# ria8651/octree-tracer

Measured on AMD Instinct MI355X. Metric: Mrays/sec at 1920x1080, depth-16 SVO; achieved HBM GB/s vs peak, higher is better.
Workload: dtype f32+u32

## Files before the change

octree-tracer_amd/csrc/svo_abi.cpp:

```cpp
#include <hip/hip_runtime.h>

#include <cmath>
#include <cstdio>
#include <cstring>
#include <new>
#include <string>
#include <vector>

#include "svo_ctx.h"

int svo_fail(svo_ctx *ctx, int code, const char *what) {
    if (ctx) ctx->err = what;
    return code;
}

int svo_fail_hip(svo_ctx *ctx, hipError_t e, const char *what) {
    if (ctx) ctx->err = std::string(what) + ": " + hipGetErrorString(e);
    return SVO_ERR_HIP;
}

namespace {

constexpr size_t kScanCapacity = 1024000;

// ... 4 lines not shown
    do {                                                     \
        hipError_t e_ = (expr);                              \
        if (e_ != hipSuccess) return fail_hip(ctx, e_, #expr); \
    } while (0)

int bind(svo_ctx *ctx) {
    HIP_TRY(ctx, hipSetDevice(ctx->device));
    return SVO_OK;
}

int order_after_last_write(svo_ctx *ctx) {
    svo_node_store *st = ctx->store;
    if (st->last_write && st->last_writer != ctx->stream) HIP_TRY(ctx, hipStreamWaitEvent(ctx->stream, st->last_write, 0));
    return SVO_OK;
}

int note_write(svo_ctx *ctx, bool on_stream) {
    svo_node_store *st = ctx->store;
    st->version++;
    if (on_stream) {
        if (!st->last_write) HIP_TRY(ctx, hipEventCreateWithFlags(&st->last_write, hipEventDisableTiming));
        HIP_TRY(ctx, hipEventRecord(st->last_write, ctx->stream));
        st->last_writer = ctx->stream;
    }
    return SVO_OK;
}

void release_store(svo_ctx *ctx) {
    svo_node_store *st = ctx->store;
    ctx->store = nullptr;
    ctx->nodes = nullptr;
    ctx->capacity = 0;
    ctx->top_version = 0;
    if (!st || --st->refs > 0) return;
    (void)hipSetDevice(st->device);
    if (st->nodes && st->owned) (void)hipFree(st->nodes);
    if (st->last_write) (void)hipEventDestroy(st->last_write);
    delete st;
}

void adopt_store(svo_ctx *ctx, svo_node_store *st) {
    ctx->store = st;
    ctx->nodes = st->nodes;
    ctx->capacity = st->capacity;
    ctx->top_version = 0;
}

int ensure_top_table(svo_ctx *ctx) {
    if (ctx->top_version == ctx->store->version) return SVO_OK;
    int rc = order_after_last_write(ctx);
    if (rc) return rc;
    HIP_TRY(ctx, svo::launch_build_top_table(ctx->nodes, (uint32_t)ctx->capacity, ctx->top_table, ctx->stream));
    ctx->top_version = ctx->store->version;
    return SVO_OK;
}

bool cull_worthwhile(const svo_ctx *ctx) {
    if (ctx->cull_mode == 0) return false;
    const float *ci = ctx->uniforms.camera_inverse;
    const double w = ci[15];
    if (!(fabs(w) > 1e-20)) return false;
    const double o[3] = {ci[12] / w, ci[13] / w, ci[14] / w};
    if (!(fabs(o[0]) > 1.001 || fabs(o[1]) > 1.001 || fabs(o[2]) > 1.001)) return false;
    if (ctx->cull_mode == 1) return true;
    constexpr int NX = 12, NY = 8;
    int miss = 0;
    for (int j = 0; j < NY; j++)
        for (int i = 0; i < NX; i++) {
            const double cx = (i + 0.5) / NX * 2.0 - 1.0, cy = -((j + 0.5) / NY * 2.0 - 1.0);
            double d4[4];
            for (int r = 0; r < 4; r++) d4[r] = ci[r] * cx + ci[4 + r] * cy + ci[8 + r] + ci[12 + r];
            if (!(fabs(d4[3]) > 1e-20)) return false;
            double t0 = -1e300, t1 = 1e300;
            for (int k = 0; k < 3; k++) {
                const double d = d4[k] / d4[3] - o[k];
                if (d == 0.0) {
                    if (fabs(o[k]) > 1.0) t1 = -1e300;
                    continue;
// ... 12 lines not shown
    bool count_rays = false;
    int sched_slot = 0;
    const uint8_t *skip = nullptr;
    svo_hit *shadow_out = nullptr;
};

int trace_launch(svo_ctx *ctx, const svo::WorkDesc &work, const float *rays, svo_hit *hits, const TraceOpts &opt) {
    int rc = bind(ctx);
    if (rc) return rc;
    const bool want_stack = ctx->variant != SVO_VARIANT_RESTART && ctx->tree_depth <= (uint32_t)svo::stack_max_depth(true);
    if (want_stack) {
        rc = ensure_top_table(ctx);
        if (rc) return rc;
    } else {
        rc = order_after_last_write(ctx);
        if (rc) return rc;
    }
    svo::WorkDesc wd = work;
    auto magic = [](uint32_t d) -> uint32_t { return d <= 1u ? 0u : (uint32_t)(0x100000000ull / d) + 1u; };
    wd.magic_bpr = magic(wd.bpr);
    wd.magic_bprect = magic(wd.bprect);
    wd.magic_tiles_x = magic(wd.tiles_x);
    svo::TraceArgs a{};
    a.nodes = ctx->nodes;
    a.n_words = (uint32_t)ctx->capacity;
    a.top_table = ctx->top_table;
    a.u = ctx->uniforms;
    a.work = wd;
    a.rays = rays;
    a.hits = hits;
    a.aux_t = opt.aux_t;
    a.status = ctx->status;
    a.refill_min = ctx->refill_min;
    a.cam_shortcut = ctx->cam_shortcut ? 1u : 0u;
    a.debug = ctx->debug_buf;
    a.skip = opt.skip;
    const bool counting = (work.mode != 2 || opt.count_rays) && !(ctx->uniforms.flags & SVO_F_PAUSE_ADAPTIVE);
    a.count_nodes = counting ? ctx->nodes : nullptr;
    const bool debug_hits = (ctx->uniforms.flags & SVO_F_PAUSE_ADAPTIVE) && (ctx->uniforms.flags & SVO_F_SHOW_HITS);
    const bool stack = want_stack && !debug_hits;
    a.shadow_hits = stack ? opt.shadow_out : nullptr;
    const uint32_t n_strips = (wd.n_items + 63u) / 64u;
    const bool schedule = ctx->schedule && n_strips <= svo::kMaxScheduledStrips;
    svo_ctx::Sched &sc = ctx->sched[opt.sched_slot & 1];
    const bool cull = stack && schedule && wd.mode != 2 && hits != nullptr && cull_worthwhile(ctx);
    const bool filtered = stack && schedule && (opt.skip != nullptr || cull);
    if (stack && schedule) {
        if (sc.cap < n_strips) {
            HIP_TRY(ctx, hipStreamSynchronize(ctx->stream));
            if (sc.cost) (void)hipFree(sc.cost);
            if (sc.cls_now) (void)hipFree(sc.cls_now);
            if (sc.order) (void)hipFree(sc.order);
            if (sc.balance) (void)hipFree(sc.balance);
            sc = svo_ctx::Sched{};
            size_t want = n_strips < 4096 ? 4096 : n_strips;
            HIP_TRY(ctx, hipMalloc((void **)&sc.cost, want + 32 + svo::kOrderHistWords * sizeof(uint32_t)));
            HIP_TRY(ctx, hipMalloc((void **)&sc.cls_now, want + 32 + svo::kOrderHistWords * sizeof(uint32_t)));
            HIP_TRY(ctx, hipMalloc((void **)&sc.order, (2 * want + 8 * (svo::kCostClasses + 8) + 8) * sizeof(uint32_t)));
            HIP_TRY(ctx, hipMalloc((void **)&sc.balance, svo::kBalanceWords * sizeof(uint32_t)));
            sc.cap = want;
        }
        if (sc.valid && memcmp(&sc.key, &wd, sizeof(wd)) != 0) sc.valid = false;
        if (!sc.valid) {
            uint32_t init[svo::kBalanceWords] = {};
            for (uint32_t k = 0; k <= 8; k++) init[k] = k * 8192u;
            HIP_TRY(ctx, hipMemcpyAsync(sc.balance, init, sizeof(init), hipMemcpyHostToDevice, ctx->stream));
            sc.balance_frames = 0;
        }
        a.balance = ctx->list_balance ? sc.balance : nullptr;
        a.order_cap = svo::order_list_cap(wd, n_strips);
        if (filtered) {
            if (opt.skip)
                HIP_TRY(ctx, svo::launch_schedule_skipping(opt.skip, wd.n_items, sc.valid ? sc.cost : nullptr, sc.cls_now, sc.order, n_strips,
                                                           a.order_cap, ctx->stream));
            else
                HIP_TRY(ctx, svo::launch_schedule_culling(a, sc.valid ? sc.cost : nullptr, sc.cls_now, sc.order, n_strips, a.order_cap,
                                                          ctx->stream));
            a.order = sc.order;
            sc.order_filtered = true;
        } else {
            a.order = (sc.valid && !sc.order_filtered) ? sc.order : nullptr;
        }
    }
    svo::LaunchInfo li{};
    li.variant = stack ? SVO_VARIANT_STACK : SVO_VARIANT_RESTART;
    li.grid_blocks = ctx->grid_blocks;
    li.num_cus = ctx->num_cus;
    li.strip_items = ctx->strip_items;
    li.deep_stack = ctx->tree_depth > (uint32_t)svo::stack_max_depth(false);
    li.occupancy = ctx->occupancy;
    if (stack && ctx->defer_items < wd.n_items) {
        HIP_TRY(ctx, hipStreamSynchronize(ctx->stream));
        if (ctx->defer_buf) (void)hipFree(ctx->defer_buf);
        ctx->defer_buf = nullptr;
        ctx->frame_parity = 0;
        ctx->defer_items = 0;
        size_t want = wd.n_items < (1u << 16) ? (1u << 16) : wd.n_items;
        HIP_TRY(ctx, hipMalloc((void **)&ctx->defer_buf, (svo::kCounterWords + 2 * (want + 1)) * sizeof(uint32_t)));
        HIP_TRY(ctx, hipMemsetAsync(ctx->defer_buf, 0, (svo::kCounterWords + 2 * (want + 1)) * sizeof(uint32_t), ctx->stream));
        ctx->defer_items = want;
    }
    li.counters = ctx->defer_buf;
    li.work_counter = ctx->defer_buf;
    if (ctx->defer_buf) {
        uint32_t *lists = ctx->defer_buf + svo::kCounterWords;
        const size_t stride = ctx->defer_items + 1;
        li.defer = lists + (ctx->frame_parity ? stride : 0);
        li.next_defer_count = lists + (ctx->frame_parity ? 0 : stride);
    }
    const size_t slot = ctx->ev_slots ? (ctx->ev_count % ctx->ev_slots) : 0;
    const bool timed = ctx->ev_slots && opt.sched_slot == 0;
    if (timed) HIP_TRY(ctx, hipEventRecord(ctx->ev[2 * slot], ctx->stream));
    HIP_TRY(ctx, svo::launch_trace(a, li, ctx->stream));
    if (timed) {
        HIP_TRY(ctx, hipEventRecord(ctx->ev[2 * slot + 1], ctx->stream));
        ctx->ev_count++;
    }
    if (stack) {
        const bool same_input = (wd.mode != 2 || opt.sched_slot == 1) && sc.built_nodes_version == ctx->store->version &&
                                memcmp(&sc.built_uniforms, &ctx->uniforms, sizeof(svo_uniforms)) == 0 && sc.age < 64;
        const bool moving = sc.have_prev && memcmp(&sc.prev_uniforms, &ctx->uniforms, sizeof(svo_uniforms)) != 0;
        const bool fed_back = a.balance != nullptr && a.order != nullptr && !filtered;
        const bool rebuild = schedule && (!sc.valid || (sc.order_filtered && !filtered) || (!same_input && sc.age + 1 >= ctx->sched_period) ||
                                          (same_input && sc.floored && !moving) || (same_input && fed_back && sc.balance_frames < 16u));
        const bool shares_only = rebuild && sc.valid && same_input && fed_back && sc.balance_frames < 16u && !(sc.order_filtered && !filtered) &&
                                 !(sc.floored && !moving);
        const bool floor_now = rebuild && !filtered && moving && ctx->motion_floor != 0u && wd.mode == 0 && wd.n_rects == 1u;
        HIP_TRY(ctx, svo::launch_post(a, li, rebuild ? sc.cost : nullptr, sc.order, n_strips, svo::order_list_cap(wd, n_strips),
                                      rebuild && !filtered, ctx->stream, floor_now ? sc.cls_now : nullptr, ctx->motion_floor,
                                      (fed_back && (!same_input || sc.balance_frames < 16u)) ? sc.balance_frames + 1u : 0u, shares_only));
        if (fed_back) sc.balance_frames++;
        if (rebuild && !filtered) sc.floored = floor_now;
        sc.prev_uniforms = ctx->uniforms;
        sc.have_prev = true;
        ctx->frame_parity ^= 1;
        if (rebuild) {
            if (!filtered) sc.order_filtered = false;
            sc.key = wd;
            sc.valid = true;
            sc.age = 0;
            sc.built_uniforms = ctx->uniforms;
            sc.built_nodes_version = ctx->store->version;
        } else if (schedule) {
            sc.age++;
        }
    }
// ... 223 lines not shown
    HIP_TRY(ctx, hipStreamSynchronize(ctx->stream));
    if (ctx->comm_stream) HIP_TRY(ctx, hipStreamSynchronize(ctx->comm_stream));
    HIP_TRY(ctx, hipFree(device_ptr));
    return SVO_OK;
}

int svo_buffer_read(svo_ctx *ctx, const void *device_ptr, void *host_out, size_t bytes) {
    if (!ctx || ((!device_ptr || !host_out) && bytes)) return SVO_ERR_ARG;
    int rc = bind(ctx);
    if (rc || bytes == 0) return rc;
    HIP_TRY(ctx, hipMemcpyAsync(host_out, device_ptr, bytes, hipMemcpyDeviceToHost, ctx->stream));
    HIP_TRY(ctx, hipStreamSynchronize(ctx->stream));
    return SVO_OK;
}

int svo_ctx_create(int hip_device, svo_ctx **out) {
    if (!out) return SVO_ERR_ARG;
    *out = nullptr;
    int n = 0;
    if (hipGetDeviceCount(&n) != hipSuccess || n <= 0) return SVO_ERR_NO_DEVICE;
    if (hip_device < 0 || hip_device >= n) return SVO_ERR_ARG;
    svo_ctx *ctx = new (std::nothrow) svo_ctx();
    if (!ctx) return SVO_ERR_HIP;
    ctx->device = hip_device;
    hipError_t e = hipSetDevice(hip_device);
    hipDeviceProp_t prop;
    if (e == hipSuccess) e = hipGetDeviceProperties(&prop, hip_device);
    if (e == hipSuccess) {
        ctx->num_cus = prop.multiProcessorCount;
        e = hipStreamCreateWithFlags(&ctx->own_stream, hipStreamNonBlocking);
    }
    if (e == hipSuccess) e = hipMalloc((void **)&ctx->top_table, (svo::kTopEntries + svo::kTopAuxEntries) * sizeof(uint32_t));
    if (e == hipSuccess) e = hipMalloc((void **)&ctx->status, sizeof(uint32_t));
    if (e == hipSuccess) e = hipMemset(ctx->status, 0, sizeof(uint32_t));
    if (e != hipSuccess) {
        svo_ctx_destroy(ctx);
        return SVO_ERR_HIP;
    }
    ctx->stream = ctx->own_stream;
    *out = ctx;
    return SVO_OK;
}

int svo_ctx_destroy(svo_ctx *ctx) {
    if (!ctx) return SVO_OK;
    (void)hipSetDevice(ctx->device);
    if (ctx->stream) (void)hipStreamSynchronize(ctx->stream);
    svo_comm_release(ctx);
    release_store(ctx);
    if (ctx->top_table) (void)hipFree(ctx->top_table);
    if (ctx->status) (void)hipFree(ctx->status);
    if (ctx->defer_buf) (void)hipFree(ctx->defer_buf);
    for (auto &sc : ctx->sched) {
        if (sc.cost) (void)hipFree(sc.cost);
        if (sc.cls_now) (void)hipFree(sc.cls_now);
        if (sc.order) (void)hipFree(sc.order);
    }
    for (void *p : {ctx->shade_hits, ctx->shade_aux, ctx->shade_rays, ctx->shade_shadow, ctx->shade_skip, ctx->scatter_buf})
        if (p) (void)hipFree(p);
    if (ctx->scan_sub) (void)hipFree(ctx->scan_sub);
    if (ctx->stage) (void)hipFree(ctx->stage);
    for (hipEvent_t e : ctx->ev) (void)hipEventDestroy(e);
    if (ctx->own_stream) (void)hipStreamDestroy(ctx->own_stream);
    delete ctx;
    return SVO_OK;
}

int svo_ctx_set_stream(svo_ctx *ctx, void *hip_stream, int use_own) {
    if (!ctx) return SVO_ERR_ARG;
    int rc = bind(ctx);
    if (rc) return rc;
    HIP_TRY(ctx, hipStreamSynchronize(ctx->stream));
    ctx->stream = use_own ? ctx->own_stream : (hipStream_t)hip_stream;
    return SVO_OK;
}

int svo_set_option(svo_ctx *ctx, int option, int64_t value) {
    if (!ctx) return SVO_ERR_ARG;
    switch (option) {
        case SVO_OPT_VARIANT:
            if (value != SVO_VARIANT_RESTART && value != SVO_VARIANT_STACK) return fail(ctx, SVO_ERR_ARG, "unknown variant");
            ctx->variant = (int)value;
            return SVO_OK;
        case SVO_OPT_TIMING: {
// ... 445 lines not shown
```

octree-tracer_amd/csrc/svo_ctx.h:

```cpp
#pragma once
#include <cstdlib>
#include <hip/hip_runtime.h>

#include <cstdint>
#include <string>
#include <vector>

#include "svo_device.h"
#include "svo_hip.h"

struct svo_node_store {
    int device = 0;
    uint32_t *nodes = nullptr;
    size_t capacity = 0;
    bool owned = false;
    int refs = 1;
    uint64_t version = 1;
    hipEvent_t last_write = nullptr;
    hipStream_t last_writer = nullptr;
};

struct svo_ctx {
    int device = 0;
    int num_cus = 256;
    hipStream_t own_stream = nullptr;
    hipStream_t stream = nullptr;
    svo_node_store *store = nullptr;
    uint32_t *nodes = nullptr;
    size_t capacity = 0;
    uint64_t top_version = 0;
    uint32_t *top_table = nullptr;
    int cull_mode = 2;
    bool cam_shortcut = true;
    void *comm = nullptr;
    int comm_world = 0, comm_rank = 0;
    hipStream_t comm_stream = nullptr;
    hipEvent_t comm_ready = nullptr, comm_done = nullptr;
    bool gathers_issued = false;
    uint32_t *status = nullptr;
    uint32_t *defer_buf = nullptr;
    size_t defer_items = 0;
    uint32_t *scan_sub = nullptr, *scan_unsub = nullptr;
    size_t scan_capacity = 0;
    void *stage = nullptr;
    size_t stage_bytes = 0;
    svo_uniforms uniforms{};
    bool have_uniforms = false;
    int variant = SVO_VARIANT_STACK;
    int grid_blocks = 0;
    int occupancy[16] = {};
    uint32_t refill_min = 32;
    bool scan_clears = false;
    int fused_shadows = 2;
    void *scatter_buf = nullptr;
    size_t scatter_bytes = 0;
    uint32_t prio_steps = 0;
    uint32_t block_w_log2 = 3;
    uint32_t tree_depth = 16;
    struct Sched {
        uint8_t *cost = nullptr;
        uint8_t *cls_now = nullptr;
        uint32_t *order = nullptr;
        uint32_t *balance = nullptr;
        uint32_t balance_frames = 0;
        size_t cap = 0;
        bool valid = false;
// ... 30 lines not shown
```

octree-tracer_amd/csrc/svo_device.h:

```cpp
#pragma once
#include <hip/hip_runtime.h>
#include <stdint.h>

#include "svo_hip.h"

namespace svo {

constexpr uint32_t kVoxelOffset = 134217728u;
constexpr uint32_t kMaxDescent = 31;
constexpr int kTopLevels = 3;
constexpr int kTopEntries = 1 << (3 * kTopLevels);
constexpr int kTopAuxEntries = 8 + 64;
constexpr int kPathBits = 23;
#ifndef SVO_COUNTER_STRIDE
#define SVO_COUNTER_STRIDE 16416
#endif
constexpr int kCounterStride = SVO_COUNTER_STRIDE;
constexpr int kCounterWords = 64 * kCounterStride;


struct WorkDesc {
    uint32_t mode;
    uint32_t x0, y0;
    uint32_t w, h;
    uint32_t bw_log2;
    uint32_t bpr;
    uint32_t bprect;
    uint32_t n_rects;
    uint32_t tiles_x;
    uint32_t first_tile, tile_stride;
    uint32_t n_items;
    uint32_t magic_bpr, magic_bprect, magic_tiles_x;
};

struct TraceArgs {
    const uint32_t *nodes;
    uint32_t n_words;
    const uint32_t *top_table;
    svo_uniforms u;
    WorkDesc work;
    const float *rays;
    svo_hit *hits;
    uint32_t *rgba;
    float *aux_t;
    uint32_t *status;
    uint32_t refill_min;
    uint32_t cam_shortcut;
    uint32_t *count_nodes;
    const uint32_t *order;
    uint32_t order_cap;
    uint32_t *debug;
    const uint8_t *skip;
    uint32_t *balance;
    svo_hit *shadow_hits;
};

struct LaunchInfo {
    int variant;
    int grid_blocks;
    int num_cus;
    int *occupancy;
    bool deep_stack;
    uint32_t strip_items;
    uint32_t *counters;
    uint32_t *work_counter;
    uint32_t *defer;
    uint32_t *next_defer_count;
};

hipError_t launch_build_top_table(const uint32_t *nodes, uint32_t n_words, uint32_t *top_table,
                                  hipStream_t stream);
hipError_t launch_trace(const TraceArgs &args, const LaunchInfo &li, hipStream_t stream);
int stack_max_depth(bool deep);
constexpr uint32_t kMaxScheduledStrips = 1u << 20;
#ifndef SVO_COST_SHIFT
#define SVO_COST_SHIFT 2
#endif
constexpr uint32_t kCostShift = SVO_COST_SHIFT, kCostClasses = 128u >> SVO_COST_SHIFT;
constexpr uint32_t kOrderHistWords = 64 * kCostClasses;
constexpr uint32_t kBalanceHead = 32, kBalanceSlots = 4096, kBalanceWords = kBalanceHead + kBalanceSlots;
// ... 26 lines not shown
```

octree-tracer_amd/csrc/svo_kernels.hip:

```cpp
#include <hip/hip_runtime.h>

#include "svo_device.h"
#include "svo_trace_fn.h"

#ifndef SVO_WALK_STOP
#define SVO_WALK_STOP 1
#endif
#ifndef SVO_TOP_IN_LDS
#define SVO_TOP_IN_LDS 1
#endif
#ifndef SVO_WALK_TRIPS
#define SVO_WALK_TRIPS 1
#endif
#ifndef SVO_WALK_ASM
#define SVO_WALK_ASM 1
#endif
#ifndef SVO_WALK_LUT
#define SVO_WALK_LUT 2
#endif
#ifndef SVO_WALK_LUT_CNT
#define SVO_WALK_LUT_CNT 1
#endif
#ifndef SVO_DBG_LIGHT
#define SVO_DBG_LIGHT 0
#endif
#ifndef SVO_CAM_SCALAR
#define SVO_CAM_SCALAR 0
#endif
#ifndef SVO_WAVES_PER_SIMD_CNT
#define SVO_WAVES_PER_SIMD_CNT 6
#endif
#ifndef SVO_WAVES_PER_SIMD
#define SVO_WAVES_PER_SIMD 7
#endif

namespace svo {


__device__ __forceinline__ uint32_t count_add(uint32_t *nodes, uint32_t p, uint32_t word, uint32_t n) {
    while ((word & 15u) < 15u) {
        const uint32_t add = min(n, 15u - (word & 15u));
        const uint32_t seen = atomicCAS(&nodes[p], word, word + add);
        if (seen == word) return (word & 15u) + add;
        word = seen;
    }
    return 15u;
}

template <bool RUNS_ONLY = false>
__device__ __forceinline__ uint32_t visit_groups(uint32_t n_words, uint32_t p, uint32_t word) {
    const bool need = p < n_words && (word & 15u) < 15u;
    const uint64_t needmask = __ballot(need);
    if (!needmask) return 0u;
    const uint32_t lane = __lane_id();
    if (RUNS_ONLY) {
        const uint32_t pm = need ? p : 0xFFFFFFFFu;
        const uint32_t under = (uint32_t)__builtin_amdgcn_update_dpp(-1, (int)pm, 0x138, 0xF, 0xF, false);
        const bool head = need && under != pm;
        const uint64_t stop = ((((uint64_t)__ballot(head) | ~needmask) >> 1) | (1ull << 63)) >> lane;
        return head ? (uint32_t)__builtin_ctzll(stop) + 1u : 0u;
// ... 137 lines not shown
        entry = (((uint32_t)top_levels + 1u) << 27) | (tn & 0x07FFFFFFu);
    }
    table[cell] = entry;
    uint32_t at = (uint32_t)kTopEntries;
    for (int k = 1; k < top_levels; k++) {
        if (cell < (1u << (3 * k))) {
            const uint32_t kx = (cell >> (2 * k)) & ((1u << k) - 1u), ky = (cell >> k) & ((1u << k) - 1u), kz = cell & ((1u << k) - 1u);
            uint32_t g = 0;
            for (int lvl = 1; lvl <= k && g != 0xFFFFFFFFu; lvl++) {
                const int sh = k - lvl;
                const uint32_t child = (((kx >> sh) & 1u) << 2) | (((ky >> sh) & 1u) << 1) | ((kz >> sh) & 1u);
                const uint32_t tn = load_word(rs, g + child) >> 4;
                g = tn >= kVoxelOffset ? 0xFFFFFFFFu : tn;
            }
            table[at + cell] = g;
        }
        at += 1u << (3 * k);
    }
}


__device__ __forceinline__ const TraceArgs &fresh_args() {
    auto p = (const __attribute__((address_space(4))) char *)__builtin_amdgcn_kernarg_segment_ptr();
    asm volatile("" : "+s"(p));
    return *(const TraceArgs *)p;
}

template <int BLOCK, int NS, int K, bool CNT>
struct StackLds {
    static constexpr int top = SVO_TOP_IN_LDS != 0 ? (1 << (3 * K)) : 0;
    static constexpr int lut = top;
    static constexpr int pools = lut + 64;
    static constexpr int counting = pools + (BLOCK / 64) * (kPoolWords * 64);
    static constexpr int stacks = counting + (CNT ? (BLOCK / 64) * kCountQueue + kSatTags + (1 << (3 * K)) / 8 : 0);
    static constexpr int total = stacks + NS * BLOCK;
};
#if defined(__HIP_DEVICE_COMPILE__) && !defined(__gfx950__)
#error "svo_kernels.hip is written for gfx950: the walk relies on its handling of LDS accesses beyond the allocation and on v_rcp_f32 + one Newton step being the IEEE reciprocal (tools/rcptest_gpu.hip)"
#endif

template <int BLOCK, int NS, int K, bool GE, bool DBG, bool CNT, bool SHD>
__global__ __launch_bounds__(BLOCK, NS > 12 ? 4 : (CNT ? SVO_WAVES_PER_SIMD_CNT : ((SHD || (DBG && SVO_DBG_LIGHT == 0)) ? 6 : SVO_WAVES_PER_SIMD))) void trace_stack_kernel(TraceArgs a, uint32_t strip_items,
                                                               uint32_t *work_counter, uint32_t *defer) {
    constexpr bool DBGH = DBG && SVO_DBG_LIGHT == 0;
    constexpr int D = kPathBits;
    constexpr int SBASE = K + 2;
    constexpr int SMAX = K + 1 + NS;
    static_assert(SMAX <= D - 1, "stack deeper than the path codes");
    constexpr int TBL = 1 << (3 * K);
    constexpr bool kTopInLds = SVO_TOP_IN_LDS != 0;
    using Lds = StackLds<BLOCK, NS, K, CNT>;
    constexpr int kLutWords = 64;
    constexpr int LOFF = Lds::lut;
    constexpr int TOFF = Lds::pools;
    constexpr bool kLut = SVO_WALK_LUT != 0 && NS <= 12 && (!CNT || SVO_WALK_LUT_CNT != 0);
    constexpr int SOFF = Lds::stacks;
    static_assert(Lds::total == SOFF + NS * BLOCK, "the ancestor stacks are the last LDS region (see StackLds)");
    static_assert(D == 23, "2^D + code must be an f32 with unit spacing");
    constexpr float kScale = (float)(1 << (D - 1));
    constexpr float kInvScale = 1.0f / kScale;
    constexpr float kMagic = (float)(1 << D);
    constexpr float kNudge = 0.000002f * kScale;
    float shadow_d0 = 0.0f, shadow_d1 = 0.0f, shadow_d2 = 0.0f;
    float sDr0 = 1.0f, sDr1 = 1.0f, sDr2 = 1.0f, sY0 = 1.0f, sY1 = 1.0f, sY2 = 1.0f;
    float sS0 = 1.0f, sS1 = 1.0f, sS2 = 1.0f;
    if (SHD) {
        auto uni = [](float x) { return __uint_as_float(__builtin_amdgcn_readfirstlane(__float_as_uint(x))); };
        float sun[3];
        sun_direction(a.u, sun);
// ... 70 lines not shown
        const uint32_t n0 = (i0 && slot0 != 0xFFFFFFFFu) ? cq[slot0] >> 27 : rec0 >> 27;
        const uint32_t n1 = (i1 && slot1 != 0xFFFFFFFFu) ? cq[slot1] >> 27 : rec1 >> 27;
        const uint32_t f0 = i0 ? __hip_atomic_load(a.count_nodes + p0, __ATOMIC_RELAXED, __HIP_MEMORY_SCOPE_AGENT) : 15u;
        const uint32_t f1 = i1 ? __hip_atomic_load(a.count_nodes + p1, __ATOMIC_RELAXED, __HIP_MEMORY_SCOPE_AGENT) : 15u;
        const bool t0 = (f0 & 15u) < 15u, t1 = (f1 & 15u) < 15u;
        const uint32_t a0 = min(n0, 15u - (f0 & 15u)), a1 = min(n1, 15u - (f1 & 15u));
        uint32_t s0 = f0, s1 = f1;
        if (t0) s0 = atomicCAS(&a.count_nodes[p0], f0, f0 + a0);
        if (t1) s1 = atomicCAS(&a.count_nodes[p1], f1, f1 + a1);
        uint32_t c0 = !t0 ? 15u : (s0 == f0 ? (f0 & 15u) + a0 : 16u), c1 = !t1 ? 15u : (s1 == f1 ? (f1 & 15u) + a1 : 16u);
        if (c0 == 16u) c0 = count_add(a.count_nodes, p0, s0, n0);
        if (c1 == 16u) c1 = count_add(a.count_nodes, p1, s1, n1);
        if (i0 && c0 == 15u) sat_tags[sat_slot(p0)] = p0;
        if (i1 && c1 == 15u) sat_tags[sat_slot(p1)] = p1;
        cq_n = 0u;
    };
    auto cq_push = [&](bool mine, uint32_t p, uint32_t word) {
        const uint32_t n = visit_groups<true>(a.n_words, p, mine ? word : 15u);
        const uint64_t m = __ballot(n != 0u);
        if (!m) return;
#ifndef SVO_COUNT_FLUSH_AT
#define SVO_COUNT_FLUSH_AT (kCountQueue - 64)
#endif
        if (cq_n > (uint32_t)(SVO_COUNT_FLUSH_AT)) {
            if (DBGH) dbg_desc_rounds += 1u;
            const uint64_t c_f0 = DBGH ? __builtin_amdgcn_s_memtime() : 0ull;
            cq_flush();
            if (DBGH && lane == 0u) dbg_desc_lanes += (uint32_t)(__builtin_amdgcn_s_memtime() - c_f0);
        }
        if (n) cq[cq_n + __builtin_amdgcn_mbcnt_hi((uint32_t)(m >> 32), __builtin_amdgcn_mbcnt_lo((uint32_t)m, 0u))] = p | (min(n, 15u) << 27);
        cq_n += (uint32_t)__popcll(m);
    };

    if (kTopInLds) {
        for (uint32_t i = tid; i < (uint32_t)TBL; i += BLOCK) lds[i] = a.top_table[i];
    }
    if (kLut && tid < (uint32_t)kLutWords) {
        uint32_t sp3 = 0u;
#pragma unroll
        for (int j = 0; j < 6; j++) sp3 |= ((tid >> j) & 1u) << (3 * j);
        lds[LOFF + tid] = __float_as_uint((float)sp3);
    }
    if (kTopInLds || kLut) __syncthreads();

    const uint32_t n_items = a.work.n_items;
    const uint32_t wave_id = __builtin_amdgcn_readfirstlane((blockIdx.x * BLOCK + tid) >> 6);

    constexpr uint32_t kShards = 8, kShardStride = (uint32_t)kCounterStride;
    constexpr uint32_t kSubs = 8;
    static_assert(kShards * kSubs == 64, "the stealing probe reads one counter per lane");
    const uint32_t n_strips = (n_items + strip_items - 1) / strip_items;
    const uint32_t *order = a.order;
    uint32_t home = (blockIdx.x % kShards) * kSubs + (blockIdx.x / kShards) % kSubs;
    uint32_t pend = 0;
    uint32_t next, strip_end;
    auto entry_of = [=](uint32_t sh, uint32_t k) -> uint32_t {
        if (order) return k < order[sh] ? order[kShards + sh * a.order_cap + k] : 0xFFFFFFFFu;
        const uint32_t cand = (((k >> 4) * kShards + sh) << 4) | (k & 15u);
        return cand < n_strips ? cand : 0xFFFFFFFFu;
    };
    {
        const uint32_t my_rank = (blockIdx.x / kShards) * (uint32_t)(BLOCK / 64) + __builtin_amdgcn_readfirstlane(tid >> 6);
        const uint32_t s0 = __builtin_amdgcn_readfirstlane(entry_of(blockIdx.x % kShards, my_rank));
        if (s0 != 0xFFFFFFFFu) {
            next = s0 * strip_items;
            strip_end = min(next + strip_items, n_items);
        } else {
            pend = 0x00FFFFFFu;
            next = strip_end = 0xFFFFFFFEu;
        }
    }
    uint32_t pool_n = 0, pool_i = 0;
    uint32_t t_begin = 0, t_dry = 0;
    uint32_t n_rounds = 0, dbg_active = 0, dbg_iters = 0, dbg_refills = 0, dbg_gens = 0;
    uint64_t c_mark = 0;
    if (DBG) t_begin = (uint32_t)__builtin_amdgcn_s_memrealtime();
// ... 345 lines not shown
                          [trips] "+s"(trips), [sv] "=&s"(saved)
                        : [m0] "v"(mu0), [m1] "v"(mu1), [m2] "v"(mu2), [rs] "s"(rs_asm), [row] "s"((uint32_t)(BLOCK * 4))
                        : "vcc", "scc", "memory");
                }
            } else
            while ((int32_t)key >= 0 && (!kWalkTrips || trips != 0u)) {
                if (kWalkTrips) trips -= 1u;
                nidx = w >> 4;
                sp += (uint32_t)(BLOCK * 4);
                if (kWalkTrips) asm("" : "+v"(sp));
                lds_at(sp) = nidx;
#if defined(SVO_DUMMY_WALK_S) || defined(SVO_DUMMY_WALK_F)
                {
#ifdef SVO_DUMMY_WALK_S
                    for (int i_ = 0; i_ < SVO_DUMMY_WALK_S; i_++) { uint32_t t_; asm volatile("v_bfe_u32 %0, %1, 1, 30" : "=v"(t_) : "v"(mu0)); }
#endif
#ifdef SVO_DUMMY_WALK_F
                    for (int i_ = 0; i_ < SVO_DUMMY_WALK_F; i_++) { uint32_t t_; asm volatile("v_add_f32 %0, 1.0, %1" : "=v"(t_) : "v"(mu0)); }
#endif
                }
#endif
                read_word();
            }
            sh = __float_as_uint(__uint_as_float(sh) + 1.0f);
            if (CNT && kWalkAsm && kLut) satm |= __builtin_bitreverse32(satb) >> ((sh + (uint32_t)(32 - D)) & 31u);
            const bool below = kWalkTrips && __uint_as_float(sh) < kMagic + (float)(D - SMAX);
            if (kWalkTrips && !kWalkStops) w = below ? 0u : w;
            leaf_off = off;
            leaf_w = w;
            if (kWalkStops) stf *= ((w >> 4) != kVoxelOffset || below) ? 0.25f : 0.5f;
            else stf *= 0.5f;
            };

    constexpr bool CAM = !CNT;
    constexpr bool kCamScalar = SVO_CAM_SCALAR != 0 && NS <= 12;
    uint32_t camv = 0;
    uint32_t cam_rows[NS] = {}, cam_leaf_off = 0, cam_leaf_w = 0, cam_sh = 0, cam_mu0 = 0, cam_mu1 = 0, cam_mu2 = 0;
    bool cam_ok = false;
    if (CAM && a.cam_shortcut && a.work.mode != 2) {
        const RayIn r0 = gen_ray(a.u, 0u, 0u);
        if (in_bounds(r0.px, r0.py, r0.pz)) {
            mu0 = entry_magic<GE>(r0.px * kScale);
            mu1 = entry_magic<GE>(r0.py * kScale);
            mu2 = entry_magic<GE>(r0.pz * kScale);
            stf = ST_DESC;
            restart_at(1u);
            descend();
            uint32_t v = lane < (uint32_t)NS ? (uint32_t)lds_at(colbase + (kRb + (uint32_t)SBASE + lane) * kRow) : 0u;
            v = lane == (uint32_t)NS ? leaf_off : v;
            v = lane == (uint32_t)NS + 1u ? leaf_w : v;
            v = lane == (uint32_t)NS + 2u ? sh : v;
            camv = v;
            if (kCamScalar) {
#pragma unroll
                for (int l = 0; l < NS; l++) cam_rows[l] = (uint32_t)__builtin_amdgcn_readlane((int)v, l);
                cam_leaf_off = (uint32_t)__builtin_amdgcn_readfirstlane((int)leaf_off);
                cam_leaf_w = (uint32_t)__builtin_amdgcn_readfirstlane((int)leaf_w);
                cam_sh = (uint32_t)__builtin_amdgcn_readfirstlane((int)sh);
                cam_mu0 = (uint32_t)__builtin_amdgcn_readfirstlane((int)mu0);
                cam_mu1 = (uint32_t)__builtin_amdgcn_readfirstlane((int)mu1);
                cam_mu2 = (uint32_t)__builtin_amdgcn_readfirstlane((int)mu2);
            }
            cam_ok = (uint32_t)D - sh_of((uint32_t)__builtin_amdgcn_readfirstlane(sh)) >= (uint32_t)(SBASE + 2);
            stf = ST_IDLE;
        }
    }

    {
        uint32_t *const bal = fresh_args().balance;
        if (bal != nullptr && blockIdx.x == 0u && tid == 0u) {
            bal[9] = (uint32_t)__builtin_amdgcn_s_memrealtime();
        }
    }
    if (DBG) {
        uint32_t *const ev = fresh_args().debug + 16u * 16384u + 16u * wave_id;
        if (lane == 0u) ev[0] = (uint32_t)__builtin_amdgcn_s_memrealtime();
        if (lane == 0u) ev[15] = (((uint32_t)__builtin_amdgcn_s_getreg((4 - 1) << 11 | 0 << 6 | 20)) << 16) | (uint32_t)__builtin_amdgcn_s_getreg((16 - 1) << 11 | 0 << 6 | 4);
    }
    for (;;) {
        if (DBGH) c_mark = __builtin_amdgcn_s_memtime();
        if (DBG) n_rounds += 1;
        if (DBGH) {
            const uint32_t nd = (uint32_t)__popcll(__ballot(sabs(stf) == ST_DESC));
            (void)nd;
            if (!CNT) dbg_desc_rounds += nd ? 1u : 0u;
        }
        if (sabs(stf) == ST_DESC) {
            descend();
        }
        if (DBGH) {
            const uint64_t now = __builtin_amdgcn_s_memtime();
            c_desc += (uint32_t)(now - c_mark);
            c_mark = now;
        }
        uint64_t act = __ballot(sabs(stf) >= ST_LEAF);
        const uint32_t n_idle = 64u - (uint32_t)__popcll(act);
        if (n_idle >= a.refill_min) {
            if (next == 0xFFFFFFFEu && pool_n == 0u) {
                const uint64_t c_w0 = DBG ? __builtin_amdgcn_s_memtime() : 0ull;
// ... 104 lines not shown
                        }
#endif
                        next = strip_end = 0xFFFFFFFEu;
                    }
                    if (DBG && next == 0xFFFFFFFFu && t_dry == 0) t_dry = (uint32_t)__builtin_amdgcn_s_memrealtime() | 1u;
                    if (DBGH) c_gen += (uint32_t)(__builtin_amdgcn_s_memtime() - c_g0);
                }
                if (sabs(stf) == ST_PENDING) flush_record(true);
                if (SHD) act = __ballot(sabs(stf) >= ST_LEAF);
                if (!(sabs(stf) >= ST_LEAF)) {
                    const uint64_t idle = ~act;
                    const uint32_t rank = __builtin_amdgcn_mbcnt_hi((uint32_t)(idle >> 32),
                                                                    __builtin_amdgcn_mbcnt_lo((uint32_t)idle, 0u));
                    if (rank < pool_n) {
                        const uint32_t e = pool_i + rank;
                        P0 = __uint_as_float(pool[0 * 64 + e]);
                        P1 = __uint_as_float(pool[1 * 64 + e]);
                        P2 = __uint_as_float(pool[2 * 64 + e]);
                        Dr0 = __uint_as_float(pool[3 * 64 + e]);
                        Dr1 = __uint_as_float(pool[4 * 64 + e]);
                        Dr2 = __uint_as_float(pool[5 * 64 + e]);
                        Y0 = recip_rn(Dr0);
                        Y1 = recip_rn(Dr1);
                        Y2 = recip_rn(Dr2);
                        S0 = copysign_bits(1.0f, Dr0);
                        S1 = copysign_bits(1.0f, Dr1);
                        S2 = copysign_bits(1.0f, Dr2);
                        dist = __uint_as_float(pool[6 * 64 + e]);
                        out = pool[7 * 64 + e];
                        tcur = 0.0f;
                        stepsf = 0.0f;
                        nmf = 0.0f;
                        if (CAM && cam_ok && dist == 0.0f) {
                            if (kCamScalar) {
#pragma unroll
                                for (int l = 0; l < NS; l++) lds_at(colbase + (kRb + (uint32_t)SBASE + (uint32_t)l) * kRow) = cam_rows[l];
                                leaf_off = cam_leaf_off;
                                leaf_w = cam_leaf_w;
                                sh = cam_sh;
                                mu0 = cam_mu0; mu1 = cam_mu1; mu2 = cam_mu2;
                            } else {
                                const uint32_t sh0 = (uint32_t)__builtin_amdgcn_readlane((int)camv, NS + 2), L0 = (uint32_t)D - sh_of(sh0);
                                for (uint32_t l = 0; l < (uint32_t)NS && l + (uint32_t)SBASE <= L0; l++)
                                    lds_at(colbase + (kRb + (uint32_t)SBASE + l) * kRow) = (uint32_t)__builtin_amdgcn_readlane((int)camv, (int)l);
                                leaf_off = (uint32_t)__builtin_amdgcn_readlane((int)camv, NS);
                                leaf_w = (uint32_t)__builtin_amdgcn_readlane((int)camv, NS + 1);
                                sh = sh0;
                                mu0 = entry_magic<GE>(P0); mu1 = entry_magic<GE>(P1); mu2 = entry_magic<GE>(P2);
                            }
                            stf = (kWalkStops && (leaf_w >> 4) != kVoxelOffset) ? ST_PENDING : ST_LEAF;
                        } else {
                            mu0 = entry_magic<GE>(P0);
                            mu1 = entry_magic<GE>(P1);
                            mu2 = entry_magic<GE>(P2);
                            stf = ST_DESC;
                            if (CNT) satm = 0u;
                            restart_at(1u);
                        }
                    }
                }
                const uint32_t took = min(SHD ? 64u - (uint32_t)__popcll(act) : n_idle, pool_n);
                pool_i += took;
                pool_n -= took;
                act = __ballot(sabs(stf) >= ST_LEAF);
            }
            if (SHD && !more) {
                if (sabs(stf) == ST_PENDING) flush_record(true);
                act = __ballot(sabs(stf) >= ST_LEAF);
            }
            if (act == 0ull && pool_n == 0u && next == 0xFFFFFFFFu) break;
        }

        if (DBGH) {
            dbg_active += (uint32_t)__popcll(__ballot(sabs(stf) == ST_LEAF));
            const uint64_t now = __builtin_amdgcn_s_memtime();
            c_refill += (uint32_t)(now - c_mark);
            c_mark = now;
        }
        if (CNT) {
            const bool at_leaf = sabs(stf) == ST_LEAF && !(kWalkTrips && __uint_as_float(sh) < kMagic + (float)(D - SMAX));
            const uint64_t c_c0 = DBGH ? __builtin_amdgcn_s_memtime() : 0ull;
            if (__ballot(at_leaf) != 0ull) {
// ... 901 lines not shown
```

Before: 9987.

## Cache camera-origin descent image across frames and share it through LDS

Before, every wave of every workgroup re-walked the tree from the camera origin at kernel start to seed rays that start at the eye. Now the host keeps a small device image of that descent, keyed on node-store version, uniforms and depth mode. When the key matches, workgroups load it straight into LDS and re-read the leaf word from nodes. Otherwise only the first wave per workgroup computes it and block 0 writes it back. The top-table staging into LDS is also widened to 16-byte loads. This adds an extra barrier and LDS words per block, a static assert guards occupancy, and caching results across calls depends on the key being complete.

```diff
diff --git a/octree-tracer_amd/csrc/svo_abi.cpp b/octree-tracer_amd/csrc/svo_abi.cpp
--- a/octree-tracer_amd/csrc/svo_abi.cpp
+++ b/octree-tracer_amd/csrc/svo_abi.cpp
@@ -60,6 +60,7 @@
     ctx->nodes = nullptr;
     ctx->capacity = 0;
     ctx->top_version = 0;
+    ctx->cam_version = 0;
     if (!st || --st->refs > 0) return;
     (void)hipSetDevice(st->device);
     if (st->nodes && st->owned) (void)hipFree(st->nodes);
@@ -72,6 +73,7 @@
     ctx->nodes = st->nodes;
     ctx->capacity = st->capacity;
     ctx->top_version = 0;
+    ctx->cam_version = 0;
 }
 
 int ensure_top_table(svo_ctx *ctx) {
@@ -150,7 +152,6 @@
     a.aux_t = opt.aux_t;
     a.status = ctx->status;
     a.refill_min = ctx->refill_min;
-    a.cam_shortcut = ctx->cam_shortcut ? 1u : 0u;
     a.debug = ctx->debug_buf;
     a.skip = opt.skip;
     const bool counting = (work.mode != 2 || opt.count_rays) && !(ctx->uniforms.flags & SVO_F_PAUSE_ADAPTIVE);
@@ -158,6 +159,12 @@
     const bool debug_hits = (ctx->uniforms.flags & SVO_F_PAUSE_ADAPTIVE) && (ctx->uniforms.flags & SVO_F_SHOW_HITS);
     const bool stack = want_stack && !debug_hits;
     a.shadow_hits = stack ? opt.shadow_out : nullptr;
+    const bool deep = ctx->tree_depth > (uint32_t)svo::stack_max_depth(false);
+    const bool cam = stack && ctx->cam_shortcut && wd.mode != 2 && !counting && wd.n_items != 0;
+    const bool cam_same = cam && ctx->cam_version == ctx->store->version && ctx->cam_deep == deep &&
+                          memcmp(&ctx->cam_uniforms, &ctx->uniforms, sizeof(svo_uniforms)) == 0;
+    a.cam_shortcut = !ctx->cam_shortcut ? 0u : (cam_same ? 2u : 1u);
+    a.cam_image = cam ? ctx->cam_image : nullptr;
     const uint32_t n_strips = (wd.n_items + 63u) / 64u;
     const bool schedule = ctx->schedule && n_strips <= svo::kMaxScheduledStrips;
     svo_ctx::Sched &sc = ctx->sched[opt.sched_slot & 1];
@@ -205,7 +212,7 @@
     li.grid_blocks = ctx->grid_blocks;
     li.num_cus = ctx->num_cus;
     li.strip_items = ctx->strip_items;
-    li.deep_stack = ctx->tree_depth > (uint32_t)svo::stack_max_depth(false);
+    li.deep_stack = deep;
     li.occupancy = ctx->occupancy;
     if (stack && ctx->defer_items < wd.n_items) {
         HIP_TRY(ctx, hipStreamSynchronize(ctx->stream));
@@ -230,6 +237,11 @@
     const bool timed = ctx->ev_slots && opt.sched_slot == 0;
     if (timed) HIP_TRY(ctx, hipEventRecord(ctx->ev[2 * slot], ctx->stream));
     HIP_TRY(ctx, svo::launch_trace(a, li, ctx->stream));
+    if (cam && !cam_same) {
+        ctx->cam_version = ctx->store->version;
+        ctx->cam_uniforms = ctx->uniforms;
+        ctx->cam_deep = deep;
+    }
     if (timed) {
         HIP_TRY(ctx, hipEventRecord(ctx->ev[2 * slot + 1], ctx->stream));
         ctx->ev_count++;
@@ -519,6 +531,7 @@
     }
     if (e == hipSuccess) e = hipMalloc((void **)&ctx->top_table, (svo::kTopEntries + svo::kTopAuxEntries) * sizeof(uint32_t));
     if (e == hipSuccess) e = hipMalloc((void **)&ctx->status, sizeof(uint32_t));
+    if (e == hipSuccess) e = hipMalloc((void **)&ctx->cam_image, 32 * sizeof(uint32_t));
     if (e == hipSuccess) e = hipMemset(ctx->status, 0, sizeof(uint32_t));
     if (e != hipSuccess) {
         svo_ctx_destroy(ctx);
@@ -537,6 +550,7 @@
     release_store(ctx);
     if (ctx->top_table) (void)hipFree(ctx->top_table);
     if (ctx->status) (void)hipFree(ctx->status);
+    if (ctx->cam_image) (void)hipFree(ctx->cam_image);
     if (ctx->defer_buf) (void)hipFree(ctx->defer_buf);
     for (auto &sc : ctx->sched) {
         if (sc.cost) (void)hipFree(sc.cost);
diff --git a/octree-tracer_amd/csrc/svo_ctx.h b/octree-tracer_amd/csrc/svo_ctx.h
--- a/octree-tracer_amd/csrc/svo_ctx.h
+++ b/octree-tracer_amd/csrc/svo_ctx.h
@@ -32,6 +32,10 @@
     uint32_t *top_table = nullptr;
     int cull_mode = 2;
     bool cam_shortcut = true;
+    uint32_t *cam_image = nullptr;
+    uint64_t cam_version = 0;
+    svo_uniforms cam_uniforms{};
+    bool cam_deep = false;
     void *comm = nullptr;
     int comm_world = 0, comm_rank = 0;
     hipStream_t comm_stream = nullptr;
diff --git a/octree-tracer_amd/csrc/svo_device.h b/octree-tracer_amd/csrc/svo_device.h
--- a/octree-tracer_amd/csrc/svo_device.h
+++ b/octree-tracer_amd/csrc/svo_device.h
@@ -46,6 +46,7 @@
     uint32_t *status;
     uint32_t refill_min;
     uint32_t cam_shortcut;
+    uint32_t *cam_image;
     uint32_t *count_nodes;
     const uint32_t *order;
     uint32_t order_cap;
diff --git a/octree-tracer_amd/csrc/svo_kernels.hip b/octree-tracer_amd/csrc/svo_kernels.hip
--- a/octree-tracer_amd/csrc/svo_kernels.hip
+++ b/octree-tracer_amd/csrc/svo_kernels.hip
@@ -23,9 +23,6 @@
 #endif
 #ifndef SVO_DBG_LIGHT
 #define SVO_DBG_LIGHT 0
-#endif
-#ifndef SVO_CAM_SCALAR
-#define SVO_CAM_SCALAR 0
 #endif
 #ifndef SVO_WAVES_PER_SIMD_CNT
 #define SVO_WAVES_PER_SIMD_CNT 6
@@ -229,9 +226,13 @@
     static constexpr int lut = top;
     static constexpr int pools = lut + 64;
     static constexpr int counting = pools + (BLOCK / 64) * (kPoolWords * 64);
-    static constexpr int stacks = counting + (CNT ? (BLOCK / 64) * kCountQueue + kSatTags + (1 << (3 * K)) / 8 : 0);
+    static constexpr int cam_words = CNT ? 0 : (NS + 4 + 3) / 4 * 4;
+    static constexpr int cam = counting + (CNT ? (BLOCK / 64) * kCountQueue + kSatTags + (1 << (3 * K)) / 8 : 0);
+    static constexpr int stacks = cam + cam_words;
     static constexpr int total = stacks + NS * BLOCK;
 };
+static_assert(StackLds<256, 12, 3, false>::total * 4 <= 18 * 1280, "the default trace instantiation loses its seventh workgroup per CU");
+static_assert(StackLds<256, 12, 3, false>::cam % 4 == 0 && StackLds<256, 18, 3, false>::cam % 4 == 0, "the camera image is read 16 bytes at a time");
 #if defined(__HIP_DEVICE_COMPILE__) && !defined(__gfx950__)
 #error "svo_kernels.hip is written for gfx950: the walk relies on its handling of LDS accesses beyond the allocation and on v_rcp_f32 + one Newton step being the IEEE reciprocal (tools/rcptest_gpu.hip)"
 #endif
@@ -368,8 +369,19 @@
         cq_n += (uint32_t)__popcll(m);
     };
 
+    constexpr bool CAM = !CNT;
+    constexpr int CAMOFF = Lds::cam;
+    const uint32_t cam_mode = (CAM && a.work.mode != 2) ? a.cam_shortcut : 0u;
+    typedef uint32_t u32x4 __attribute__((ext_vector_type(4)));
+    static_assert(TBL % 4 == 0, "the top table is staged 16 bytes at a time");
     if (kTopInLds) {
-        for (uint32_t i = tid; i < (uint32_t)TBL; i += BLOCK) lds[i] = a.top_table[i];
+        for (uint32_t i = tid; i < (uint32_t)TBL / 4u; i += BLOCK) ((u32x4 *)lds)[i] = ((const u32x4 *)a.top_table)[i];
+    }
+    if (CAM && cam_mode == 2u && tid >= (uint32_t)(BLOCK - Lds::cam_words / 4)) {
+        const uint32_t j = tid - (uint32_t)(BLOCK - Lds::cam_words / 4);
+        u32x4 v = ((const u32x4 *)a.cam_image)[j];
+        if (j == 0u && v.w != 0u) v.y = a.nodes[v.x >> 2];
+        ((u32x4 *)lds)[CAMOFF / 4 + j] = v;
     }
     if (kLut && tid < (uint32_t)kLutWords) {
         uint32_t sp3 = 0u;
@@ -377,7 +389,7 @@
         for (int j = 0; j < 6; j++) sp3 |= ((tid >> j) & 1u) << (3 * j);
         lds[LOFF + tid] = __float_as_uint((float)sp3);
     }
-    if (kTopInLds || kLut) __syncthreads();
+    if (kTopInLds || kLut || cam_mode == 2u) __syncthreads();
 
     const uint32_t n_items = a.work.n_items;
     const uint32_t wave_id = __builtin_amdgcn_readfirstlane((blockIdx.x * BLOCK + tid) >> 6);
@@ -789,39 +801,36 @@
             else stf *= 0.5f;
             };
 
-    constexpr bool CAM = !CNT;
-    constexpr bool kCamScalar = SVO_CAM_SCALAR != 0 && NS <= 12;
-    uint32_t camv = 0;
-    uint32_t cam_rows[NS] = {}, cam_leaf_off = 0, cam_leaf_w = 0, cam_sh = 0, cam_mu0 = 0, cam_mu1 = 0, cam_mu2 = 0;
-    bool cam_ok = false;
-    if (CAM && a.cam_shortcut && a.work.mode != 2) {
-        const RayIn r0 = gen_ray(a.u, 0u, 0u);
-        if (in_bounds(r0.px, r0.py, r0.pz)) {
-            mu0 = entry_magic<GE>(r0.px * kScale);
-            mu1 = entry_magic<GE>(r0.py * kScale);
-            mu2 = entry_magic<GE>(r0.pz * kScale);
-            stf = ST_DESC;
-            restart_at(1u);
-            descend();
-            uint32_t v = lane < (uint32_t)NS ? (uint32_t)lds_at(colbase + (kRb + (uint32_t)SBASE + lane) * kRow) : 0u;
-            v = lane == (uint32_t)NS ? leaf_off : v;
-            v = lane == (uint32_t)NS + 1u ? leaf_w : v;
-            v = lane == (uint32_t)NS + 2u ? sh : v;
-            camv = v;
-            if (kCamScalar) {
-#pragma unroll
-                for (int l = 0; l < NS; l++) cam_rows[l] = (uint32_t)__builtin_amdgcn_readlane((int)v, l);
-                cam_leaf_off = (uint32_t)__builtin_amdgcn_readfirstlane((int)leaf_off);
-                cam_leaf_w = (uint32_t)__builtin_amdgcn_readfirstlane((int)leaf_w);
-                cam_sh = (uint32_t)__builtin_amdgcn_readfirstlane((int)sh);
-                cam_mu0 = (uint32_t)__builtin_amdgcn_readfirstlane((int)mu0);
-                cam_mu1 = (uint32_t)__builtin_amdgcn_readfirstlane((int)mu1);
-                cam_mu2 = (uint32_t)__builtin_amdgcn_readfirstlane((int)mu2);
-            }
-            cam_ok = (uint32_t)D - sh_of((uint32_t)__builtin_amdgcn_readfirstlane(sh)) >= (uint32_t)(SBASE + 2);
-            stf = ST_IDLE;
-        }
-    }
+    if (CAM && cam_mode == 1u) {
+        if (__builtin_amdgcn_readfirstlane(tid) < 64u) {
+            uint32_t v = 0u;
+            const RayIn r0 = gen_ray(a.u, 0u, 0u);
+            if (in_bounds(r0.px, r0.py, r0.pz)) {
+                mu0 = entry_magic<GE>(r0.px * kScale);
+                mu1 = entry_magic<GE>(r0.py * kScale);
+                mu2 = entry_magic<GE>(r0.pz * kScale);
+                stf = ST_DESC;
+                restart_at(1u);
+                descend();
+                const uint32_t shu = (uint32_t)__builtin_amdgcn_readfirstlane(sh), L = (uint32_t)D - sh_of(shu);
+                const bool below = kWalkTrips && __uint_as_float(shu) < kMagic + (float)(D - SMAX);
+                const uint32_t row = lane - 4u;
+                v = (row < (uint32_t)NS && row + (uint32_t)SBASE <= L) ? (uint32_t)lds_at(colbase + (kRb + (uint32_t)SBASE + row) * kRow) : 0u;
+                v = lane == 0u ? leaf_off : v;
+                v = lane == 1u ? leaf_w : v;
+                v = lane == 2u ? sh : v;
+                v = lane == 3u ? ((L >= (uint32_t)(SBASE + 2) && !below) ? 1u : 0u) : v;
+                stf = ST_IDLE;
+            }
+            if (lane < (uint32_t)Lds::cam_words) {
+                lds_at((CAMOFF + lane) * 4u) = v;
+                uint32_t *const img = fresh_args().cam_image;
+                if (img != nullptr && blockIdx.x == 0u) img[lane] = v;
+            }
+        }
+        __syncthreads();
+    }
+    const bool cam_ok = CAM && cam_mode != 0u && __builtin_amdgcn_readfirstlane(lds_at(CAMOFF * 4u + 12u)) != 0;
 
     {
         uint32_t *const bal = fresh_args().balance;
@@ -992,22 +1001,20 @@
                         stepsf = 0.0f;
                         nmf = 0.0f;
                         if (CAM && cam_ok && dist == 0.0f) {
-                            if (kCamScalar) {
+                            typedef __attribute__((address_space(3))) u32x4 lds_u32x4;
+                            auto img = [](int q) -> u32x4 { return *(lds_u32x4 *)(uintptr_t)((CAMOFF + 4 * q) * 4); };
 #pragma unroll
-                                for (int l = 0; l < NS; l++) lds_at(colbase + (kRb + (uint32_t)SBASE + (uint32_t)l) * kRow) = cam_rows[l];
-                                leaf_off = cam_leaf_off;
-                                leaf_w = cam_leaf_w;
-                                sh = cam_sh;
-                                mu0 = cam_mu0; mu1 = cam_mu1; mu2 = cam_mu2;
-                            } else {
-                                const uint32_t sh0 = (uint32_t)__builtin_amdgcn_readlane((int)camv, NS + 2), L0 = (uint32_t)D - sh_of(sh0);
-                                for (uint32_t l = 0; l < (uint32_t)NS && l + (uint32_t)SBASE <= L0; l++)
-                                    lds_at(colbase + (kRb + (uint32_t)SBASE + l) * kRow) = (uint32_t)__builtin_amdgcn_readlane((int)camv, (int)l);
-                                leaf_off = (uint32_t)__builtin_amdgcn_readlane((int)camv, NS);
-                                leaf_w = (uint32_t)__builtin_amdgcn_readlane((int)camv, NS + 1);
-                                sh = sh0;
-                                mu0 = entry_magic<GE>(P0); mu1 = entry_magic<GE>(P1); mu2 = entry_magic<GE>(P2);
+                            for (int q = 1; q < Lds::cam_words / 4; q++) {
+                                const u32x4 r = img(q);
+#pragma unroll
+                                for (int c = 0; c < 4; c++)
+                                    if (4 * (q - 1) + c < NS) lds_at(colbase + (kRb + (uint32_t)SBASE + (uint32_t)(4 * (q - 1) + c)) * kRow) = r[c];
                             }
+                            const u32x4 hd = img(0);
+                            leaf_off = hd.x;
+                            leaf_w = hd.y;
+                            sh = hd.z;
+                            mu0 = entry_magic<GE>(P0); mu1 = entry_magic<GE>(P1); mu2 = entry_magic<GE>(P2);
                             stf = (kWalkStops && (leaf_w >> 4) != kVoxelOffset) ? ST_PENDING : ST_LEAF;
                         } else {
                             mu0 = entry_magic<GE>(P0);
```

After: 10180 (median of 6 runs). 1.02x the previous value.
